# XunshanMan/Object-oriented-SLAM

Hardware: AMD Instinct MI355X
Metric: LM iterations/sec (cams+ellipsoids) (higher is better)
Workload: dtype f64

## Files before the change

object-oriented-slam_amd/csrc/esl_capi.hip:

```cpp
#include <algorithm>
#include <cfloat>
#include <cmath>
#include <cstdio>
#include <cstdlib>
#include <cstring>
#include <numeric>

#include "esl_graph_int.hpp"
#include "esl_graph_layout.hpp"
#include "esl_kernels_map.hpp"
#include "esl_kernels_chunk.hpp"
#include "esl_slam.hpp"
#include "esl_fixed.hpp"

namespace esl {
static thread_local std::string g_err;
void set_error(const std::string& s) { g_err = s; }
}

using namespace esl;

namespace esl {
ProfScope::ProfScope(esl_ctx* ctx, int kind) : c(ctx), slot(-1) {
  if (!c || !c->prof_on) return;
// ... 70 lines not shown
  int n = 0;
  if (hipGetDeviceCount(&n) != hipSuccess) return 0;
  return n;
}

void esl_lm_params_default(esl_lm_params* p) {
  p->max_iters = 10;
  p->max_trials = 10;
  p->tau = 1e-5;
  p->jacobian_mode = ESL_JAC_NUMERIC;
  p->numeric_delta = 1e-9;
  p->linear_solver = ESL_SOLVER_AUTO;
  p->drop_nan_bbox = 1;
  p->bbox_residual = ESL_BBOX_REPROJECTION;
  p->e3d_half_turn = 0;
}

int esl_ctx_create(int device_id, esl_ctx** out) {
  if (!out) return ESL_ERR_INVALID;
  *out = nullptr;
  int n = 0;
  if (hipGetDeviceCount(&n) != hipSuccess || n <= 0) {
    set_error("no HIP device visible: libesl_hip has no CPU fallback");
    return ESL_ERR_NO_DEVICE;
  }
  if (device_id < 0 || device_id >= n) { set_error("device id out of range"); return ESL_ERR_INVALID; }
  ESL_HIP_TRY(hipSetDevice(device_id));
  esl_ctx* c = new esl_ctx();
  c->device = device_id;
  { const char* ov = std::getenv("ESL_CF_OVERLAP"); c->sw_cf_overlap = (ov && ov[0] >= '0' && ov[0] <= '4') ? ov[0] - '0' : 4; }
  { const char* ok = std::getenv("ESL_CF_OS_KERNEL"); c->sw_cf_os_kernel = (ok && ok[0] == '0') ? 0 : 1; }
  { const char* ol = std::getenv("ESL_CF_OS_LIST"); c->sw_cf_os_list = (ol && ol[0] == '0') ? 0 : 1; }
  { const char* sp = std::getenv("ESL_CF_SWEEP"); c->sw_cf_sweep = (sp && sp[0] == '0') ? 0 : 1; }
  { const char* fp = std::getenv("ESL_CF_FWD_PARTS"); const int v = fp ? std::atoi(fp) : 0; if (v == 2 || v == 4 || v == 8) c->sw_cf_fwd_parts = v; }
  { const char* sd = std::getenv("ESL_CF_STRIDE"); const int v = sd ? std::atoi(sd) : 0; c->sw_cf_stride = (v == 16 || v == 32 || v == 48) ? v : 0; }
  auto init = [&]() -> int {
    ESL_HIP_TRY(hipStreamCreateWithFlags(&c->stream, hipStreamNonBlocking));
    ESL_HIP_TRY(hipHostMalloc((void**)&c->host_part, 16 * sizeof(double), hipHostMallocDefault));
    ESL_HIP_TRY(hipMalloc((void**)&c->dev_part, 16 * sizeof(double)));
    ESL_HIP_TRY(hipMalloc((void**)&c->chol_info, 4 * sizeof(int)));
    ESL_HIP_TRY(hipMemset(c->chol_info, 0, 4 * sizeof(int)));
    ESL_HIP_TRY(hipMalloc((void**)&c->tickets, 4 * sizeof(unsigned int)));
    ESL_HIP_TRY(hipMemset(c->tickets, 0, 4 * sizeof(unsigned int)));
    ESL_HIP_TRY(hipMalloc((void**)&c->dev_scal, 8 * sizeof(double)));
    ESL_HIP_TRY(hipEventCreateWithFlags(&c->ev_try, hipEventDisableTiming));
    ESL_HIP_TRY(hipHostMalloc(&c->host_scal, sizeof(LmScalars), hipHostMallocMapped));
    ESL_HIP_TRY(hipHostGetDevicePointer(&c->host_scal_dev, c->host_scal, 0));
    std::memset(c->host_scal, 0, sizeof(LmScalars));
    ESL_HIP_TRY(hipMalloc(&c->lm_dev, 2 * sizeof(LmCore)));
    ESL_HIP_TRY(hipMemset(c->lm_dev, 0, 2 * sizeof(LmCore)));
    ESL_HIP_TRY(hipHostMalloc(&c->lm_host, sizeof(LmHostView), hipHostMallocMapped));
    ESL_HIP_TRY(hipHostGetDevicePointer(&c->lm_host_dev, c->lm_host, 0));
    std::memset(c->lm_host, 0, sizeof(LmHostView));
    return ESL_OK;
  };
  const int rc = init();
  if (rc) { const std::string msg = g_err; esl_ctx_destroy(c); set_error(msg); return rc; }
  *out = c;
  return ESL_OK;
}

int esl_ctx_destroy(esl_ctx* c) {
  if (!c) return ESL_OK;
  (void)hipSetDevice(c->device);
  if (c->stream) (void)hipStreamSynchronize(c->stream);
  slam_sync_side(c);
// ... 763 lines not shown
```

object-oriented-slam_amd/csrc/esl_cf_plan.hpp:

```cpp
#pragma once
#include <algorithm>
#include <array>
#include <cmath>
#include <cstddef>
#include <cstdint>
#include <utility>
#include <vector>

namespace esl {

constexpr int kCfFwdCh = 16;
constexpr int kCfSyT = 128;
constexpr int kCfSegRows = 96;
constexpr int kCfMaxStride = 128;
constexpr int kCfKC = 16;
constexpr int kCfSparseMinCams = 256;

constexpr double kCfUpdFlopsPerMs = 0.83 * 79.0e9;
constexpr double kCfPairMs = (7.82 - 4.21) / (77.35e6 - 31.05e6);
constexpr double kCfSlabMs = 1.30 / 1.35e8;
constexpr double kCfStrideMargin = 0.05;
inline double cf_stride_cost(double upd_flops, double pairs, double slab) {
  return upd_flops / kCfUpdFlopsPerMs + pairs * kCfPairMs + slab * kCfSlabMs;
}
inline int cf_stride_choose(long n_o, const double* upd_flops, const double* pairs, const double* slab) {
  if (n_o < 8192) return kCfFwdCh;
  const double base = cf_stride_cost(upd_flops[0], pairs[0], slab[0]);
  int best = 1;
  double best_ms = base * (1.0 - kCfStrideMargin);
  for (int m = 2; m <= 3; ++m) {
    const double ms = cf_stride_cost(upd_flops[m - 1], pairs[m - 1], slab[m - 1]);
    if (ms < best_ms) { best = m; best_ms = ms; }
  }
  return best * kCfFwdCh;
}

struct CfSwitches {
  int sparse = -1;
  bool tperm_off = false;
  bool no_nd = false;
  int nd_min = 48;
  int stride = 0;
  int os_kernel = 1;
  int os_list = 1;
  int sweep = 1;
};

struct CfSegTables {
  int S = kCfFwdCh, nseg = 0, nw = 0;
  std::vector<int> p, o, first;
  std::vector<int> seg_start, xld, fw_off;
  std::vector<long long> xoff, boff, roff, tw_off;
  int n_fwork = 0, n_twork = 0;
  size_t xc_len = 0, p_blocks = 0, prhs_len = 0;
  double sp_flops = 0;
};
struct CfPlan : CfSegTables {
  int n_list = 0, n_chunks = 0;
  int64_t ldx = 0, ldt = 0, kpad = 0, kpad_s = 0;
  bool nd = false;
  int stride = 0, n_sep = 0, n_seg = 1;
  bool sparse = false;
  int form = 0;
  std::vector<int> os, ou;
  size_t y_len = 0;
  size_t os_npairs = 0;
  bool os_offsets = false;
  double os_flops = 0;
  bool os_list = false;
  std::vector<int> os_run, os_heads;
  size_t osm_npairs = 0, osm_row_npairs = 0, os_list_npairs = 0;
  double osm_flops = 0;
  bool sweep = false;
  std::vector<int> sl_ent;
  size_t xl_len = 0;
  bool tperm = false;
  std::vector<int> rank, unrank, kfirst;
  double upd_flops = 0;
};

inline void cf_entry_lists(int N, int nf, const std::vector<int>& start, const int* cu_start, const int* cu_obj, const int* cu_id,
                           std::vector<int>& os, std::vector<int>& ou) {
  std::vector<int> cur(start.begin(), start.end() - 1);
  os.assign((size_t)start[(size_t)N], 0); ou.assign((size_t)start[(size_t)N], 0);
  for (int sl = 0; sl < nf; ++sl)
    for (int q = cu_start[sl]; q < cu_start[sl + 1]; ++q) { const int at = cur[cu_obj[q]]++; os[(size_t)at] = sl; ou[(size_t)at] = cu_id[q]; }
}
inline CfSegTables cf_walk(int S, int N, int nf, const int* cu_start, const int* cu_obj) {
  CfSegTables t;
  const int nseg = (nf + S - 1) / S;
  t.S = S; t.nseg = nseg; t.nw = (nseg + 63) / 64;
  std::vector<int> last_seg((size_t)N, -1);
  for (int sl = 0; sl < nf; ++sl) {
    const int p = sl / S, pos = sl - p * S;
    if (pos == S - 1) continue;
    for (int q = cu_start[sl]; q < cu_start[sl + 1]; ++q) {
      const int o = cu_obj[q];
      if (last_seg[(size_t)o] != p) { last_seg[(size_t)o] = p; t.p.push_back(p); t.o.push_back(o); t.first.push_back(pos); }
    }
  }
  const size_t n_inc = t.p.size();
  const long long rows = S == kCfFwdCh ? kCfSegRows : 6 * (S - 1);
  t.seg_start.assign((size_t)nseg + 1, 0); t.xld.assign((size_t)nseg, 0); t.fw_off.assign((size_t)nseg + 1, 0);
  t.xoff.assign((size_t)nseg + 1, 0); t.boff.assign((size_t)nseg + 1, 0); t.roff.assign((size_t)nseg + 1, 0); t.tw_off.assign((size_t)nseg + 1, 0);
  for (size_t q = 0; q < n_inc; ++q) ++t.seg_start[(size_t)t.p[q] + 1];
  for (int p = 0; p < nseg; ++p) t.seg_start[(size_t)p + 1] += t.seg_start[(size_t)p];
  for (size_t q = 0; q < n_inc; ++q)
    t.sp_flops += 81.0 * (double)(q - (size_t)t.seg_start[(size_t)t.p[q]] + 1) * (6.0 * (S - 1 - t.first[q]));
// ... 61 lines not shown

inline void cf_os_sides(CfPlan& pl, const std::vector<int>& start) {
  const int S = pl.S;
  const size_t n_inc = pl.p.size();
  pl.os_run.assign(pl.os.size(), 0); pl.os_heads.assign(n_inc, 0);
  std::vector<int> cur(start.begin(), start.end() - 1);
  for (size_t q = 0; q < n_inc; ++q) {
    const int o = pl.o[q], p = pl.p[q], end = start[(size_t)o + 1];
    int k = cur[(size_t)o];
    while (k < end && pl.os[(size_t)k] / S < p) ++k;
    for (int head = -1; k < end && pl.os[(size_t)k] / S == p; ++k) {
      const int sl = pl.os[(size_t)k];
      if (sl % S == S - 1) continue;
      if (head < 0 || pl.os[(size_t)head] != sl) { head = k; ++pl.os_heads[q]; }
      ++pl.os_run[(size_t)head];
    }
    cur[(size_t)o] = k;
  }
  double both = 0, row = 0, brow = 0;
  std::vector<int> v;
  std::vector<std::pair<int, int>> byrank;
  for (int p = 0; p < pl.nseg; ++p) {
    const int q0 = pl.seg_start[(size_t)p], n = pl.seg_start[(size_t)p + 1] - q0;
    v.assign(pl.os_heads.begin() + q0, pl.os_heads.begin() + q0 + n);
    std::sort(v.begin(), v.end());
    for (int i = 0; i < n; ++i) { both += (double)v[(size_t)i] * (double)(n - i); brow += v[(size_t)i]; }
    byrank.clear();
    for (int i = 0; i < n; ++i) { const int o = pl.o[(size_t)(q0 + i)]; byrank.push_back({pl.rank.empty() ? o : pl.rank[(size_t)o], pl.os_heads[(size_t)(q0 + i)]}); }
    std::sort(byrank.begin(), byrank.end());
    for (int i = 0; i < n; ++i) row += (double)byrank[(size_t)i].second * (double)(i + 1);
  }
  pl.osm_npairs = (size_t)(both + brow); pl.osm_row_npairs = (size_t)(row + brow);
  pl.osm_flops = 2.0 * 6.0 * (81.0 * both + 9.0 * brow);
}

inline bool cf_plan_build(int N, int nf, size_t EU, const std::vector<int>& start, const int* cu_start, const int* cu_obj, const int* cu_id, bool chain_ok,
                          bool comm, size_t total_mem, const CfSwitches& sw, CfPlan& pl) {
  pl = CfPlan{};
  const size_t nfz = (size_t)nf, n_o = (size_t)9 * N;
  const int nch = (nf + kCfFwdCh - 1) / kCfFwdCh;
  pl.ldx = (int64_t)((n_o + 1 + 127) / 128 * 128);
  pl.kpad = (int64_t)((6 * nfz + kCfKC - 1) / kCfKC * kCfKC);
  pl.ldt = pl.ldx;
  pl.n_list = start[(size_t)N]; pl.n_chunks = nch;
  pl.nseg = nch; pl.nw = (nch + 63) / 64;
  if ((size_t)std::max(N, 1) * (size_t)(nch + 1) > ((size_t)1 << 28)) return false;
  cf_entry_lists(N, nf, start, cu_start, cu_obj, cu_id, pl.os, pl.ou);
  CfSegTables& seg = pl;
  if (chain_ok && nf >= kCfSparseMinCams && N > 0 && (size_t)nch * (size_t)(N + 1) <= ((size_t)1 << 28) && !sw.no_nd) {
    seg = cf_walk(kCfFwdCh, N, nf, cu_start, cu_obj);
    const double dense = (double)n_o * (double)n_o * 6.0 * (double)nfz;
    const double sparse = (double)n_o * (double)n_o * 6.0 * (double)(nfz / kCfFwdCh) + 24.0 * pl.sp_flops;
    pl.sparse = sw.sparse >= 0 ? sw.sparse != '0' : (n_o >= 2048 && sparse < 0.5 * dense);
    const double need = 8.0 * (81.0 * (double)pl.p_blocks + (double)pl.xc_len + 2.0 * (double)pl.ldt * (double)n_o +
                               2.0 * 6.0 * (double)(nfz / kCfFwdCh) * (double)pl.ldx  + 54.0 * (double)EU );
    pl.form = sw.sparse == '2' || need > 0.4 * (double)total_mem ? 2 : 1;
    if ((sw.sparse < 0 || sw.sparse == '3') && !comm) pl.form = 3;
  }
  const bool sp = pl.sparse;
  std::vector<int> first_cam;
  pl.tperm = sp && N > 0 && !sw.tperm_off;
  if (pl.tperm) {
    std::vector<int> cnt(nfz + 2, 0);
    first_cam.assign((size_t)N, nf);
    for (int o = 0; o < N; ++o) if (start[(size_t)o + 1] > start[(size_t)o]) first_cam[(size_t)o] = pl.os[(size_t)start[(size_t)o]];
    for (int o = 0; o < N; ++o) ++cnt[(size_t)first_cam[(size_t)o] + 1];
// ... 18 lines not shown
      seg = std::move(cand[want / kCfFwdCh - 1]);
    }
    if (!want) want = kCfFwdCh;
    if (want != pl.S) seg = cf_walk(want, N, nf, cu_start, cu_obj);
  }
  pl.nd = nfz >= (size_t)std::max(sw.nd_min, 2 * kCfFwdCh) && !sw.no_nd;
  if (pl.nd) {
    int sd = 16 * (int)std::max(1.0, std::floor(std::sqrt((double)nfz) / 16.0 + 0.5));
    sd = std::min(sd, kCfMaxStride);
    if (sp) sd = pl.S;
    pl.stride = sd; pl.n_sep = nf / sd; pl.n_seg = (nf + sd - 1) / sd;
  }
  if (sp) pl.kpad_s = (int64_t)((6 * (size_t)pl.n_sep + kCfKC - 1) / kCfKC * kCfKC);
  if (pl.tperm) pl.upd_flops = cf_staircase(pl.S, N, nf, pl.unrank, first_cam, pl.kfirst);
  if (sp && pl.form == 3) {
    const CfOsCounts n = cf_os_counts(pl.S, N, start, pl.os, pl.rank);
    const size_t y_recs = std::max<size_t>(pl.p.size(), 1) * (size_t)(pl.S - 1);
    pl.os_flops = 2.0 * 6.0 * (81.0 * n.prod + 9.0 * n.rhs_entries);
    pl.os_npairs = (size_t)(n.prod + n.rhs_entries);
    pl.y_len = y_recs * 54 + std::max<size_t>(nfz, 1) * 6;
    pl.os_offsets = sw.os_kernel != 0 && 54 * std::max(EU, y_recs) <= (size_t)INT32_MAX;
    cf_os_sides(pl, start);
    pl.os_list = sw.os_list != 0;
    pl.os_list_npairs = pl.os_list ? pl.osm_npairs : pl.os_npairs;
    pl.sweep = sw.sweep != 0;
    if (pl.sweep) {
      std::vector<int> cur(start.begin(), start.end() - 1);
      pl.sl_ent.assign((size_t)cu_start[nf], 0);
      for (int sl = 0; sl < nf; ++sl)
        for (int q = cu_start[sl]; q < cu_start[sl + 1]; ++q) pl.sl_ent[(size_t)q] = cur[cu_obj[q]]++;
      long long cols = 0;
      for (int x : pl.xld) cols += x;
      pl.xl_len = 6 * (size_t)cols;
    }
  }
  return true;
}

}
```

object-oriented-slam_amd/csrc/esl_cf_sweep.hpp:

```cpp
#pragma once
#include "esl_cf.hpp"

namespace esl {

constexpr int kCfSweepSI = 3 * kCfFwdCh - 1;

#define CF_LT(r, c) ((r) * ((r) + 1) / 2 + (c))
__device__ __forceinline__ void cf_chol6(double (&d)[21], double (&is)[6], bool& ok) {
#pragma unroll
  for (int j = 0; j < 6; ++j) {
    const double p = d[CF_LT(j, j)];
    ok = ok && (p > 0);
    double q = __builtin_amdgcn_rsq(p);
    q = q * (1.5 - 0.5 * p * q * q);
    q = q * (1.5 - 0.5 * p * q * q);
    is[j] = q;
    d[CF_LT(j, j)] = p * q;
#pragma unroll
    for (int r = j + 1; r < 6; ++r) d[CF_LT(r, j)] *= q;
#pragma unroll
    for (int r = j + 1; r < 6; ++r)
#pragma unroll
      for (int c = j + 1; c <= r; ++c) d[CF_LT(r, c)] -= d[CF_LT(r, j)] * d[CF_LT(c, j)];
  }
}

static __global__ __launch_bounds__(64) void k_cf_twist(int nf_all, int stride, const double* __restrict__ Hcc, double lambda,
                                                        const double* __restrict__ Lfac, const double* __restrict__ Gfac,
                                                        double* __restrict__ Pm, double* __restrict__ Qm, int* __restrict__ info) {
  __shared__ double sH[kCfSweepSI * 36], sG[kCfSweepSI * 36], sL[kCfSweepSI * 21];
  const int lane = threadIdx.x;
  const int beg = (int)blockIdx.x * stride;
  const int len = ((beg + stride - 1 < nf_all) ? beg + stride - 1 : nf_all) - beg;
  if (len <= 0) return;
  {
    constexpr int kQ = (kCfSweepSI * 36 + 63) / 64, kL = (kCfSweepSI * 21 + 63) / 64;
    double th[kQ], tg[kQ], tl[kL];
#pragma unroll
// ... 365 lines not shown
          for (int q = 0; q < 6; ++q) t += P[a * 6 + q] * d[q];
          sv[(ii * 6 + a) * 64 + lane] = t;
        }
      }
      if (on) {
        const bool rmw = __any(s_first < s_last && s_first < p0 + hl && p0 < s_last) != 0;
#pragma unroll
        for (int q0 = 0; q0 < CH * 6; q0 += 8) {
          double t[8], old[8];
#pragma unroll
          for (int e = 0; e < 8; ++e) t[e] = sv[((q0 + e < hl * 6) ? q0 + e : 0) * 64 + lane];
          if (rmw) {
#pragma unroll
            for (int e = 0; e < 8; ++e) {
              const int q = q0 + e, pos = p0 + q / 6;
              old[e] = (q < hl * 6 && pos >= s_first && pos < s_last) ? dst[(size_t)pos * dstep + q % 6] : 0.0;
            }
          } else {
#pragma unroll
            for (int e = 0; e < 8; ++e) old[e] = 0.0;
          }
#pragma unroll
          for (int e = 0; e < 8; ++e) {
            const int q = q0 + e, pos = p0 + q / 6;
            if (q < hl * 6 && pos < s_last) dst[(size_t)pos * dstep + q % 6] = (pos >= s_first) ? old[e] + t[e] : t[e];
          }
        }
      }
      __builtin_amdgcn_wave_barrier();
    }
  }
}

static __global__ __launch_bounds__(64) void k_cf_wxo(int stride, const int* __restrict__ sl_start, const int* __restrict__ sl_ent,
                                                      const int* __restrict__ sl_obj, const double* __restrict__ V, const double* __restrict__ vy,
                                                      const double* __restrict__ xo, double* __restrict__ z) {
  __shared__ double red[64];
  const int i = blockIdx.x, lane = threadIdx.x;
  if (i % stride == stride - 1) return;
  const int l = lane < 54 ? lane : 0, b = l / 6;
  const int qa = sl_start[i], qb = sl_start[i + 1];
  double s = 0;
  for (int q = qa; q < qb; q += 4) {
    double v[4], w[4];
#pragma unroll
    for (int e = 0; e < 4; ++e) {
      const int qq = (q + e < qb) ? q + e : qa;
      v[e] = V[(size_t)sl_ent[qq] * 54 + l];
      w[e] = xo[(size_t)9 * sl_obj[qq] + b];
    }
#pragma unroll
    for (int e = 0; e < 4; ++e) if (q + e < qb) s += v[e] * w[e];
  }
  red[lane] = s;
  __builtin_amdgcn_wave_barrier();
  if (lane < 6) {
    double t = 0;
#pragma unroll
    for (int bb = 0; bb < 9; ++bb) t += red[6 * bb + lane];
    z[(size_t)i * 6 + lane] = vy[(size_t)i * 6 + lane] - t;
  }
}
static __global__ __launch_bounds__(64) void k_cf_z_fwd(int nf_all, int stride, const double* __restrict__ Mm, double* __restrict__ z) {
  __shared__ double sM[kCfSweepSI * 36], sz[kCfSweepSI * 6];
  const int lane = threadIdx.x;
  const int beg = (int)blockIdx.x * stride;
// ... 33 lines not shown
```

object-oriented-slam_amd/csrc/esl_ctx.hpp:

```cpp
#pragma once
#include <hip/hip_runtime.h>

#include <cstdint>
#include <string>
#include <type_traits>
#include <vector>

#include "../../include/esl.h"
#include "esl_cf_plan.hpp"
#include "esl_math.hpp"

namespace esl {

void set_error(const std::string& s);
#define ESL_HIP_TRY(expr)                                                                         \
  do {                                                                                            \
    hipError_t _e = (expr);                                                                       \
    if (_e != hipSuccess) {                                                                       \
      esl::set_error(std::string(#expr) + ": " + hipGetErrorString(_e));                          \
      return ESL_ERR_HIP;                                                                         \
    }                                                                                             \
  } while (0)

struct DevGraph {
// ... 192 lines not shown
  void* lm_dev = nullptr;
  void* lm_host = nullptr;
  void* lm_host_dev = nullptr;
  void* host_scal = nullptr;
  void* host_scal_dev = nullptr;
  bool sys_combined = false;
  void* comm = nullptr;
  int comm_ranks = 1, comm_rank = 0;
  bool comm_replicated = false;
  esl_host_allreduce_fn host_allreduce = nullptr;
  void* host_user = nullptr;
  double* host_stage = nullptr;
  double* dev_gather = nullptr;
  double* host_gather = nullptr;
  double* Linv_ws = nullptr;
  double* z_ws = nullptr;
  int64_t S_lda = 0;
  bool cf_chain_ok = false;
  bool cf_ready = false;
  bool cf_unavailable = false;
  esl::CfPlan cf_plan;
  int *cf_oe_start = nullptr, *cf_oe_u = nullptr, *cf_oe_slot = nullptr, *cf_od_start = nullptr, *cf_od_edge = nullptr, *cf_oe_cst = nullptr;
  double *cf_Linv = nullptr, *cf_M = nullptr, *cf_N = nullptr, *cf_V = nullptr, *cf_vy = nullptr, *cf_z = nullptr;
  double *cf_B = nullptr, *cf_Lfac = nullptr, *cf_G = nullptr;
  double *cf_Zt = nullptr, *cf_Hs = nullptr, *cf_Bs = nullptr, *cf_LfacS = nullptr, *cf_GS = nullptr, *cf_LiS = nullptr, *cf_MS = nullptr,
         *cf_NS = nullptr, *cf_R = nullptr;
  double *cf_Xt = nullptr, *cf_T = nullptr, *cf_Linv_ws = nullptr, *cf_part = nullptr;
  int *cf_seg_start = nullptr, *cf_seg_obj = nullptr, *cf_seg_first = nullptr, *cf_cmap = nullptr, *cf_xld = nullptr, *cf_fwork = nullptr, *cf_twork = nullptr;
  unsigned long long* cf_mask = nullptr;
  long long *cf_xoff = nullptr, *cf_boff = nullptr, *cf_roff = nullptr;
  double *cf_Xc = nullptr, *cf_Xs = nullptr, *cf_P = nullptr, *cf_Prhs = nullptr, *cf_Y = nullptr, *cf_Yr = nullptr;
  double *cf_Pm = nullptr, *cf_Qm = nullptr, *cf_XL = nullptr;
  int* cf_sl_ent = nullptr;
  long long* cf_os_start = nullptr;
  int *cf_os_cnt = nullptr, *cf_os_pairs = nullptr;
  int *cf_os_run = nullptr, *cf_os_heads = nullptr;
  double* cf_Vm = nullptr;
  int *cf_rank = nullptr, *cf_unrank = nullptr, *cf_kfirst = nullptr;
  double* cf_xo_t = nullptr;
  int lm_solver_used = 0;
  bool fx_on = false;
  std::vector<uint8_t> fx_flags;
  esl::AnchGraph fx;
  char* fx_blob = nullptr; size_t fx_blob_cap = 0;
  double* fx_A = nullptr; double* fx_chi = nullptr;
  std::vector<int> fx_bb_map, fx_e3_map;
  std::vector<int> fx_grav_obj;
  bool chain_ok = false;
  esl::Scratch chain_ws;
  esl_pcg_params pcg = {1000, 8, 1e-10};
  esl_pcg_params pcg_run = {1000, 8, 1e-10};
  double* pcg_ws = nullptr; size_t pcg_ws_cap = 0;
  double* pcg_st = nullptr; double* pcg_M = nullptr;
  double* pcg_host = nullptr;
  bool pcg_ran = false;
  bool pcg_reset = true;
  void* chol_rt = nullptr;
  void* chol_prof_scope = nullptr;
  unsigned long long graph_fp = 0;
  bool repl_checked = false;
  double *chol_pack = nullptr, *chol_pack2 = nullptr;
  size_t chol_pack_len = 0;
  bool schur_attr_set = false;
  int sw_chol_dist = -1;
  bool sw_chol_overlap = true;
  int sw_cf_overlap = 4;
  int sw_cf_os_kernel = 1;
  int sw_cf_os_list = 1;
  int sw_cf_fwd_parts = 8;
  int sw_cf_sweep = 1;
  int sw_cf_stride = 0;
};
```

object-oriented-slam_amd/csrc/esl_slam.hip:

```cpp
#include "esl_slam.hpp"

#include <algorithm>
#include <array>
#include <chrono>
#include <cmath>
#include <cstdio>
#include <cstdlib>
#include <cstring>

#include "esl_cf.hpp"
#include "esl_cf_sweep.hpp"
#include "esl_chol.hpp"
#include "esl_fixed.hpp"
#include "esl_kernels_slam.hpp"
#include "esl_pcg.hpp"

namespace esl {

static __global__ __launch_bounds__(256) void k_cf_updates(DevGraph g, int nb_obj, double lambda, const double* __restrict__ objs, const double* __restrict__ bo,
                                                           const double* __restrict__ xo, double* __restrict__ objs_trial, double* __restrict__ obj_part,
                                                           const double* __restrict__ cams, const double* __restrict__ xc, const double* __restrict__ bc,
                                                           double* __restrict__ cams_trial, double* __restrict__ cam_part) {
  if ((int)blockIdx.x < nb_obj) cf_obj_update_one(g, lambda, objs, bo, xo, objs_trial, obj_part, blockIdx.x * 256 + threadIdx.x);
  else slam_cam_update_one(g, lambda, cams, xc, bc, cams_trial, cam_part, ((int)blockIdx.x - nb_obj) * 256 + threadIdx.x);
// ... 208 lines not shown
  if (c->sw_chol_overlap) {
    d.pack2 = c->chol_pack2;
    d.bcast_on = [](void* u, double* dev, size_t count, int root, hipStream_t st) { return comm_bcast((esl_ctx*)u, dev, count, root, st); };
  }
  return ESL_OK;
}
static bool cf_applicable(const esl_ctx* c) { return c->cf_chain_ok && (!c->comm || c->comm_replicated); }
static bool cf_dist(const esl_ctx* c) {
  if (!c->comm || !c->comm_replicated || c->comm_ranks < 2) return false;
  if (c->sw_chol_dist >= 0) return c->sw_chol_dist == 1;
  return 9L * c->g.n_objs >= 8192;
}
static bool chain_applicable(const esl_ctx* c) { return c->chain_ok && c->g.n_ue == 0 && !c->comm; }
static int slam_pick_solver(const esl_ctx* c) {
  const int want = c->lm.p.linear_solver;
  if (want == ESL_SOLVER_PCG) return c->comm ? -3 : ESL_SOLVER_PCG;
  if (want == ESL_SOLVER_CAMERA_CHAIN) return chain_applicable(c) ? ESL_SOLVER_CAMERA_CHAIN : -2;
  if (want == ESL_SOLVER_AUTO && c->fx_on && chain_applicable(c)) return ESL_SOLVER_CAMERA_CHAIN;
  if (want == ESL_SOLVER_REDUCED_CAMERA) return ESL_SOLVER_REDUCED_CAMERA;
  if (want == ESL_SOLVER_REDUCED_ELLIPSOID) return cf_applicable(c) ? ESL_SOLVER_REDUCED_ELLIPSOID : -1;
  if (!cf_applicable(c) || c->cf_unavailable) return ESL_SOLVER_REDUCED_CAMERA;
  const double nc = (double)c->S_n, no = 9.0 * c->g.n_objs;
  return (no * no * nc + no * no * no / 3.0 < nc * nc * nc / 3.0) ? ESL_SOLVER_REDUCED_ELLIPSOID : ESL_SOLVER_REDUCED_CAMERA;
}
static void cf_forget(esl_ctx* c) {
  c->cf_oe_start = c->cf_oe_u = c->cf_oe_slot = c->cf_oe_cst = nullptr;
  c->cf_seg_start = c->cf_seg_obj = c->cf_seg_first = c->cf_cmap = c->cf_xld = c->cf_fwork = c->cf_twork = nullptr;
  c->cf_mask = nullptr; c->cf_xoff = c->cf_boff = c->cf_roff = nullptr;
  c->cf_Linv = c->cf_M = c->cf_N = c->cf_V = c->cf_B = c->cf_Lfac = c->cf_G = c->cf_vy = c->cf_z = nullptr;
  c->cf_T = c->cf_Linv_ws = c->cf_part = nullptr;
  c->cf_Zt = c->cf_Hs = c->cf_Bs = c->cf_LfacS = c->cf_GS = c->cf_LiS = c->cf_MS = c->cf_NS = c->cf_R = nullptr;
  c->cf_Xc = c->cf_Xs = c->cf_P = c->cf_Prhs = c->cf_Xt = c->cf_Y = c->cf_Yr = nullptr;
  c->cf_os_start = nullptr; c->cf_os_cnt = c->cf_os_pairs = c->cf_os_run = c->cf_os_heads = nullptr; c->cf_Vm = nullptr;
  c->cf_Pm = c->cf_Qm = c->cf_XL = nullptr; c->cf_sl_ent = nullptr;
  c->cf_rank = c->cf_unrank = c->cf_kfirst = nullptr; c->cf_xo_t = nullptr;
  c->cf_plan = CfPlan{};
  c->cf_ready = false;
}
static int cf_ensure_impl(esl_ctx* c);
static int cf_ensure(esl_ctx* c) {
  if (c->cf_ready) return ESL_OK;
  const int rc = cf_ensure_impl(c);
  if (rc) { cf_forget(c); (void)hipGetLastError(); return rc; }
  c->cf_ready = true;
  return ESL_OK;
}
static_assert(kCfKC == kKC, "esl_cf_plan.hpp pads K to the rank-K update's chunk");
static int cf_ensure_impl(esl_ctx* c) {
  const DevGraph& g = c->g;
  const int N = g.n_objs, nfi = g.n_free_cams;
  const size_t nf = (size_t)nfi, EU = (size_t)g.n_bbox + g.n_e3d, n_o = (size_t)9 * N;
  const bool timing = std::getenv("ESL_UPLOAD_HOST_TIMING") != nullptr;
  const double t0 = timing ? now_us() : 0;
  CfSwitches sw;
  { const char* e = std::getenv("ESL_CF_SPARSE"); sw.sparse = e ? (int)(unsigned char)e[0] : -1; }
  { const char* e = std::getenv("ESL_CF_TPERM"); sw.tperm_off = e && e[0] == '0'; }
  sw.no_nd = std::getenv("ESL_CF_NO_ND") != nullptr;
  static const int nd_min = [] { const char* e = std::getenv("ESL_CF_ND_MIN"); return e ? std::atoi(e) : 48; }();
  sw.nd_min = nd_min; sw.stride = c->sw_cf_stride; sw.os_kernel = c->sw_cf_os_kernel; sw.os_list = c->sw_cf_os_list;
  sw.sweep = c->sw_cf_sweep;
  size_t free_b = 0, total_b = 0;
  if (nfi >= kCfSparseMinCams) ESL_HIP_TRY(hipMemGetInfo(&free_b, &total_b));
  CfPlan& pl = c->cf_plan;
  if (!cf_plan_build(N, nfi, EU, c->h_ue_start, c->h_cu_start, c->h_cu_obj, c->h_cu_id, c->cf_chain_ok, c->comm != nullptr, total_b, sw, pl)) {
    set_error("camera-first elimination: the (ellipsoid, camera chunk) range table of this graph exceeds 1 GB");
    return ESL_ERR_ALLOC;
  }
  const bool sp = pl.sparse, os3 = sp && pl.form == 3, osm = os3 && pl.os_list;
  const bool swp = os3 && pl.sweep;
  const int nch = pl.n_chunks, nseg = pl.nseg, nw = pl.nw, N1 = N + 1;
  const size_t n_inc = pl.p.size();
  const size_t y_recs = std::max<size_t>(n_inc, 1) * (size_t)(pl.S - 1), nb = (size_t)N * (N + 1) / 2 + N;
  const double t1 = timing ? now_us() : 0;
  BlobStage st;
  struct Up { int item; const void* src; size_t bytes; };
  std::vector<Up> ups;
  auto ship = [&](auto** dst, const auto& v) { ups.push_back({st.up(dst, v.size()), v.data(), v.size() * sizeof(v[0])}); };
  ship(&c->cf_oe_start, c->h_ue_start); ship(&c->cf_oe_u, pl.ou); ship(&c->cf_oe_slot, pl.os);
  int* d_inc = nullptr; int* d_fw_off = nullptr; long long* d_tw_off = nullptr;
  int i_inc = -1;
  if (pl.tperm) { ship(&c->cf_rank, pl.rank); ship(&c->cf_unrank, pl.unrank); ship(&c->cf_kfirst, pl.kfirst); }
  if (sp) {
    i_inc = st.up(&d_inc, 4 * n_inc); ship(&c->cf_seg_start, pl.seg_start); ship(&c->cf_xld, pl.xld);
    ship(&c->cf_xoff, pl.xoff); ship(&c->cf_boff, pl.boff); ship(&c->cf_roff, pl.roff); ship(&d_fw_off, pl.fw_off); ship(&d_tw_off, pl.tw_off);
  }
  if (osm) { ship(&c->cf_os_run, pl.os_run); ship(&c->cf_os_heads, pl.os_heads); }
  if (swp) ship(&c->cf_sl_ent, pl.sl_ent);
  st.work(&c->cf_oe_cst, (size_t)std::max(N, 1) * (nch + 1));
  if (sp) {
    st.work(&c->cf_cmap, (size_t)nseg * N1); st.work(&c->cf_mask, (size_t)N1 * nw); st.work(&c->cf_seg_obj, n_inc); st.work(&c->cf_seg_first, n_inc);
    st.work(&c->cf_fwork, 2 * (size_t)pl.n_fwork); st.work(&c->cf_twork, 3 * (size_t)pl.n_twork);
  }
  st.work(&c->cf_Linv, nf * 36); st.work(&c->cf_M, nf * 36); st.work(&c->cf_N, nf * 36); st.work(&c->cf_V, EU * 54);
  st.work(&c->cf_B, nf * 36); st.work(&c->cf_Lfac, nf * 21); st.work(&c->cf_G, nf * 36); st.work(&c->cf_vy, nf * 6); st.work(&c->cf_z, nf * 6);
  st.work(&c->cf_T, (size_t)pl.ldt * n_o); st.work(&c->cf_Linv_ws, ((n_o + kNB - 1) / kNB) * kNB * kNB);
  if (pl.tperm) st.work(&c->cf_xo_t, n_o);
  if (n_o <= 1024) st.work(&c->cf_part, (size_t)kCholMaxSplit * (size_t)pl.ldt * n_o);
  if (pl.nd) {
    const size_t ns = (size_t)std::max(pl.n_sep, 1);
    st.work(&c->cf_Zt, nf * 36); st.work(&c->cf_Hs, ns * 36); st.work(&c->cf_Bs, ns * 36); st.work(&c->cf_LfacS, ns * 21);
    st.work(&c->cf_GS, ns * 36); st.work(&c->cf_LiS, ns * 36); st.work(&c->cf_MS, ns * 36); st.work(&c->cf_NS, ns * 36);
    st.work(&c->cf_R, ns * 6 * (size_t)pl.ldx);
  }
  if (sp) {
    if (!swp) st.work(&c->cf_Xc, pl.xc_len);
    st.work(&c->cf_Xs, (size_t)pl.ldx * (size_t)pl.kpad_s);
    if (pl.form == 1) { st.work(&c->cf_P, pl.p_blocks * 81); st.work(&c->cf_Prhs, pl.prhs_len); }
    if (pl.form == 3) {
      st.work(&c->cf_Y, y_recs * 54); st.work(&c->cf_Yr, std::max<size_t>(nf, 1) * 6);
      st.work(&c->cf_os_start, nb + 1); st.work(&c->cf_os_cnt, nb); st.work(&c->cf_os_pairs, 2 * std::max<size_t>(pl.os_list_npairs, 1));
      if (osm) st.work(&c->cf_Vm, EU * 54);
      if (swp) { st.work(&c->cf_Pm, nf * 36); st.work(&c->cf_Qm, nf * 36); st.work(&c->cf_XL, std::max<size_t>(pl.xl_len, 1)); }
    }
  } else {
    st.work(&c->cf_Xt, (size_t)pl.ldx * (size_t)pl.kpad);
  }
  if (int rc = st.reserve(c->arena_solve)) return rc;
  for (const Up& u : ups) if (u.bytes) std::memcpy(st.host<char>(u.item), u.src, u.bytes);
  if (sp && n_inc) {
    int* inc = st.host<int>(i_inc);
// ... 106 lines not shown
                       c->cf_Linv, st);
  }
  int slabs(bool beside) {
    auto twist = [&](hipStream_t s) {
      hipLaunchKernelGGL(k_cf_twist, dim3((unsigned)nseg), dim3(64), 0, s, nf, st, c->Hcc, lambda, c->cf_Lfac, c->cf_G, c->cf_Pm, c->cf_Qm, c->chol_info);
    };
    hipError_t e_tw = hipSuccess;
    segment_chains([&] {
      if (!swp) return;
      if (!beside) { twist(main); return; }
      e_tw = hipEventRecord(rt.cf_ev_c, main);
      if (e_tw == hipSuccess) e_tw = hipStreamWaitEvent(rt.cf_side, rt.cf_ev_c, 0);
      if (e_tw != hipSuccess) return;
      join.armed = true;
      twist(rt.cf_side);
      e_tw = hipEventRecord(rt.cf_ev_t, rt.cf_side);
    });
    ESL_HIP_TRY(e_tw);
    if (beside) {
      ESL_HIP_TRY(hipEventRecord(rt.cf_ev_a, main));
      ESL_HIP_TRY(hipStreamWaitEvent(rt.cf_side, rt.cf_ev_a, 0));
      join.armed = true;
    }
    sep_chain(beside ? rt.cf_side : main);
    if (beside) ESL_HIP_TRY(hipEventRecord(rt.cf_ev_s, rt.cf_side));
    if (swp) {
      edge_scale(beside ? 1 : 0, main);
      if (beside) ESL_HIP_TRY(hipStreamWaitEvent(main, rt.cf_ev_t, 0));
      auto sweep = [&](auto parts) {
        hipLaunchKernelGGL((k_cf_sweep<decltype(parts)::value>), dim3((unsigned)pl.n_fwork), dim3(64), 0, main, nf, n_o, pl.n_chunks, c->cf_oe_cst, c->cf_oe_slot,
                           c->cf_V, c->cf_vy, c->cf_M, (const double*)c->cf_Zt, c->cf_Pm, c->cf_Qm, c->cf_R, ldx, st, segs(), c->cf_Y, c->cf_Yr, c->cf_XL,
                           (long long)(st == kCfFwdCh ? kCfSegRows : 6 * (st - 1)));
      };
      if (c->sw_cf_fwd_parts == 8) sweep(std::integral_constant<int, 8>{});
      else if (c->sw_cf_fwd_parts == 4) sweep(std::integral_constant<int, 4>{});
      else sweep(std::integral_constant<int, 2>{});
      return ESL_OK;
    }
    edge_scale(beside ? 1 : 0, main);
    auto forward = [&](auto parts) {
      hipLaunchKernelGGL((k_cf_forward<2, decltype(parts)::value>), dim3((unsigned)pl.n_fwork), dim3(64), 0, main, nf, n_o, pl.n_chunks, c->cf_oe_cst, c->cf_oe_slot,
                         c->cf_V, c->cf_vy, c->cf_M, c->cf_Xc, ldx, st, st - 1, (const double*)c->cf_Zt, c->cf_R, st, segs());
    };
    if (c->sw_cf_fwd_parts == 8) forward(std::integral_constant<int, 8>{});
    else if (c->sw_cf_fwd_parts == 4) forward(std::integral_constant<int, 4>{});
    else forward(std::integral_constant<int, 2>{});
    return ESL_OK;
  }
  void sep_rhs(hipStream_t s, bool sp = true) const {
    hipLaunchKernelGGL(k_cf_sep_rhs, dim3(cg, (unsigned)ns), dim3(64), 0, s, nf, n_o, st, pl.n_chunks, c->cf_oe_cst, c->cf_oe_slot, c->cf_V, c->cf_vy,
                       c->cf_G, c->cf_LiS, sp ? c->cf_Xc : c->cf_Xt, ldx, c->cf_R, sp ? (const int*)c->cf_cmap : nullptr, sp ? segs() : CfSegs{},
                       (const double*)(sp && swp ? c->cf_XL : nullptr), (long long)(st == kCfFwdCh ? kCfSegRows : 6 * (st - 1)));
  }
  void sep_forward(hipStream_t s, bool sp = true) const {
    hipLaunchKernelGGL(k_cf_forward<1>, dim3(cg), dim3(64), 0, s, ns, n_o, pl.n_chunks, c->cf_oe_cst, c->cf_oe_slot, c->cf_V, c->cf_vy,
                       c->cf_MS, sp ? c->cf_Xs : c->cf_Xt, ldx, ns, ns, (const double*)nullptr, c->cf_R, sp ? 0 : st, CfSegs{});
  }
  void products(hipStream_t s) const {
    hipLaunchKernelGGL(k_cf_seg_syrk, dim3((unsigned)pl.n_twork), dim3(256), 0, s, c->cf_twork, c->cf_seg_start, c->cf_seg_first, c->cf_xoff,
                       c->cf_xld, c->cf_Xc, c->cf_boff, c->cf_P);
    hipLaunchKernelGGL(k_cf_seg_rhs, dim3((unsigned)pl.n_fwork), dim3(64), 0, s, c->cf_fwork, c->cf_seg_start, c->cf_xoff, c->cf_xld, c->cf_Xc,
                       c->cf_roff, c->cf_Prhs);
  }
  void gather_products(long c_begin, long c_end, int accumulate) const {
    int o2b, o2e;
    const dim3 grid = block_grid(c_begin, c_end, o2b, o2e);
    hipLaunchKernelGGL(k_cf_T_gather, grid, dim3(256), 0, main, N, pl.nw, c->cf_mask, c->cf_cmap, c->cf_boff, c->cf_roff, c->cf_P, c->cf_Prhs,
// ... 794 lines not shown
```

Before: 19.62.

## Add paired-column sweep kernel so each lane solves two right-hand-side columns

Adds k_cf_sweep_pair, in which each lane handles two columns of the segment's right-hand side (128 columns per 64-lane block), plus a host-built work list mapping blocks to (segment, column group). The aim is to reuse each shared-memory load of the M/Z/P/Q 6x6 blocks across two columns, halving block count and matrix staging traffic per column. The cost is doubled register state per lane (x, acc, u, erec arrays), which may reduce occupancy or cause spills, plus extra shared memory for the interleaved sv buffer. It is enabled by default (sweep_cols=2) whenever the sweep path is active.

```diff
diff --git a/object-oriented-slam_amd/csrc/esl_capi.hip b/object-oriented-slam_amd/csrc/esl_capi.hip
--- a/object-oriented-slam_amd/csrc/esl_capi.hip
+++ b/object-oriented-slam_amd/csrc/esl_capi.hip
@@ -126,6 +126,7 @@
   { const char* ok = std::getenv("ESL_CF_OS_KERNEL"); c->sw_cf_os_kernel = (ok && ok[0] == '0') ? 0 : 1; }
   { const char* ol = std::getenv("ESL_CF_OS_LIST"); c->sw_cf_os_list = (ol && ol[0] == '0') ? 0 : 1; }
   { const char* sp = std::getenv("ESL_CF_SWEEP"); c->sw_cf_sweep = (sp && sp[0] == '0') ? 0 : 1; }
+  { const char* sc = std::getenv("ESL_CF_SWEEP_COLS"); c->sw_cf_sweep_cols = (sc && sc[0] == '1') ? 1 : 2; }
   { const char* fp = std::getenv("ESL_CF_FWD_PARTS"); const int v = fp ? std::atoi(fp) : 0; if (v == 2 || v == 4 || v == 8) c->sw_cf_fwd_parts = v; }
   { const char* sd = std::getenv("ESL_CF_STRIDE"); const int v = sd ? std::atoi(sd) : 0; c->sw_cf_stride = (v == 16 || v == 32 || v == 48) ? v : 0; }
   auto init = [&]() -> int {
diff --git a/object-oriented-slam_amd/csrc/esl_cf_plan.hpp b/object-oriented-slam_amd/csrc/esl_cf_plan.hpp
--- a/object-oriented-slam_amd/csrc/esl_cf_plan.hpp
+++ b/object-oriented-slam_amd/csrc/esl_cf_plan.hpp
@@ -10,6 +10,7 @@
 namespace esl {
 
 constexpr int kCfFwdCh = 16;
+constexpr int kCfPairCols = 128;
 constexpr int kCfSyT = 128;
 constexpr int kCfSegRows = 96;
 constexpr int kCfMaxStride = 128;
@@ -44,6 +45,7 @@
   int os_kernel = 1;
   int os_list = 1;
   int sweep = 1;
+  int sweep_cols = 2;
 };
 
 struct CfSegTables {
@@ -74,6 +76,8 @@
   bool sweep = false;
   std::vector<int> sl_ent;
   size_t xl_len = 0;
+  std::vector<int> pw_off, pwork;
+  int n_pwork = 0;
   bool tperm = false;
   std::vector<int> rank, unrank, kfirst;
   double upd_flops = 0;
@@ -201,6 +205,17 @@
   }
   pl.osm_npairs = (size_t)(both + brow); pl.osm_row_npairs = (size_t)(row + brow);
   pl.osm_flops = 2.0 * 6.0 * (81.0 * both + 9.0 * brow);
+}
+
+inline void cf_pair_work(const std::vector<int>& seg_start, std::vector<int>& pw_off, std::vector<int>& pwork) {
+  const size_t nseg = seg_start.empty() ? 0 : seg_start.size() - 1;
+  pw_off.assign(nseg + 1, 0); pwork.clear();
+  for (size_t p = 0; p < nseg; ++p) {
+    const int m = 9 * (seg_start[p + 1] - seg_start[p]) + 1;
+    const int ng = (m + kCfPairCols - 1) / kCfPairCols;
+    pw_off[p + 1] = pw_off[p] + ng;
+    for (int q = 0; q < ng; ++q) { pwork.push_back((int)p); pwork.push_back(q); }
+  }
 }
 
 inline bool cf_plan_build(int N, int nf, size_t EU, const std::vector<int>& start, const int* cu_start, const int* cu_obj, const int* cu_id, bool chain_ok,
@@ -285,6 +300,8 @@
       long long cols = 0;
       for (int x : pl.xld) cols += x;
       pl.xl_len = 6 * (size_t)cols;
+      if (sw.sweep_cols == 2) cf_pair_work(pl.seg_start, pl.pw_off, pl.pwork);
+      pl.n_pwork = (int)(pl.pwork.size() / 2);
     }
   }
   return true;
diff --git a/object-oriented-slam_amd/csrc/esl_cf_sweep.hpp b/object-oriented-slam_amd/csrc/esl_cf_sweep.hpp
--- a/object-oriented-slam_amd/csrc/esl_cf_sweep.hpp
+++ b/object-oriented-slam_amd/csrc/esl_cf_sweep.hpp
@@ -4,6 +4,7 @@
 namespace esl {
 
 constexpr int kCfSweepSI = 3 * kCfFwdCh - 1;
+constexpr int kCfPairE = 4;
 
 #define CF_LT(r, c) ((r) * ((r) + 1) / 2 + (c))
 __device__ __forceinline__ void cf_chol6(double (&d)[21], double (&is)[6], bool& ok) {
@@ -435,6 +436,283 @@
   }
 }
 
+template <int PARTS>
+static __global__ __launch_bounds__(64) void k_cf_sweep_pair(int nf_all, int n_o, int n_chunks, const int* __restrict__ oe_cst, const int* __restrict__ oe_slot,
+                                                             const double* __restrict__ V, const double* __restrict__ vy, const double* __restrict__ Mm,
+                                                             const double* __restrict__ Zt, const double* __restrict__ Pm, const double* __restrict__ Qm,
+                                                             double* __restrict__ R, long ldx, int stride, CfSegs sg, const int* __restrict__ pwork,
+                                                             double* __restrict__ Y, double* __restrict__ Yr, double* __restrict__ XL, long long xl_rows) {
+  static_assert(PARTS == 2 || PARTS == 4 || PARTS == 8, "halves, quarters or eighths of a chunk");
+  constexpr int CH = kCfFwdCh / PARTS;
+  constexpr int HC = kCfFwdCh / 2;
+  constexpr int kQ = (HC * 36 + 63) / 64;
+  constexpr int kB = 2;
+  constexpr int kE = kCfPairE;
+  static_assert(HC % CH == 0 && HC * 6 <= 64, "a part lies inside a half chunk; one load per lane stages its right-hand sides");
+  __shared__ __attribute__((aligned(16))) double sA[HC * 36], sB[HC * 36], sP[HC * 36];
+  __shared__ double sv[CH * 6 * 128];
+  __shared__ double svy[HC * 6];
+  const int lane = threadIdx.x;
+  const int seg = pwork[2 * blockIdx.x];
+  auto jc = [&](int c) { return pwork[2 * blockIdx.x + 1] * kCfPairCols + 64 * c + lane; };
+  const int ob = sg.seg_start[seg];
+  const int jr = 9 * (sg.seg_start[seg + 1] - ob);
+  const int SI = stride - 1;
+  const int beg = seg * stride;
+  const int nf = (beg + SI < nf_all) ? beg + SI : nf_all;
+  if (beg >= nf) return;
+  const int len = nf - beg;
+  const bool use_z = Zt != nullptr && seg >= 1;
+  int oc[2], ka[2], s_first[2], s_last[2], t_first[2], ecnt[2], eslot[2][kE];
+  int kind[2];
+  double* dst[2];
+  double erec[2][kE][6];
+#pragma unroll
+  for (int c = 0; c < 2; ++c) {
+    const int j = jc(c);
+    kind[c] = j < jr ? 1 : j == jr ? 2 : 0;
+    const int oi = j < jr ? j / 9 : 0, b = j - 9 * oi;
+    const int o = j < jr ? sg.seg_obj[ob + oi] : 0;
+    const int* cst = oe_cst + (size_t)o * (n_chunks + 1);
+    oc[c] = o;
+    s_first[c] = len; s_last[c] = -1; t_first[c] = len; ecnt[c] = 0; ka[c] = 0;
+#pragma unroll
+    for (int e = 0; e < kE; ++e) {
+      eslot[c][e] = -1;
+#pragma unroll
+      for (int a = 0; a < 6; ++a) erec[c][e][a] = 0.0;
+    }
+    if (kind[c] == 2) { s_first[c] = 0; s_last[c] = len - 1; }
+    else if (kind[c] == 1) {
+      const int c0 = beg / kCfFwdCh, c1 = (c0 + stride / kCfFwdCh < n_chunks) ? c0 + stride / kCfFwdCh : n_chunks;
+      const int k0 = cst[c0], kb = cst[c1];
+      if (k0 < kb) {
+        const int f = oe_slot[k0] - beg;
+        int k = kb - 1, l = oe_slot[k] - beg;
+        while (l >= len && k > k0) { --k; l = oe_slot[k] - beg; }
+        if (f < len) {
+          s_first[c] = f; s_last[c] = l; ecnt[c] = k - k0 + 1; ka[c] = k0;
+          if (ecnt[c] > kE) t_first[c] = oe_slot[k0 + kE] - beg;
+#pragma unroll
+          for (int e = 0; e < kE; ++e) {
+            const int kk = e < ecnt[c] ? k0 + e : k0;
+            eslot[c][e] = oe_slot[kk] - beg;
+            const double* src = V + ((size_t)kk * 9 + b) * 6;
+#pragma unroll
+            for (int a = 0; a < 6; ++a) erec[c][e][a] = src[a];
+          }
+        }
+      }
+    }
+    dst[c] = kind[c] == 2 ? Yr + (size_t)beg * 6 : Y + ((size_t)(ob + oi) * SI) * 54 + b * 6;
+  }
+  auto gather = [&](int h0, int p0, int hl) {
+#pragma unroll
+    for (int q = 0; q < CH * 6 * 2; ++q) sv[q * 64 + lane] = 0.0;
+    __builtin_amdgcn_wave_barrier();
+#pragma unroll
+    for (int c = 0; c < 2; ++c) {
+      if (kind[c] == 2) {
+#pragma unroll
+        for (int q = 0; q < CH * 6; ++q) sv[(2 * q + c) * 64 + lane] = (q < hl * 6) ? svy[h0 * 6 + q] : 0.0;
+      } else if (kind[c] == 1) {
+#pragma unroll
+        for (int e = 0; e < kE; ++e) {
+          const int at = eslot[c][e] - p0;
+          if (e < ecnt[c] && at >= 0 && at < hl) {
+#pragma unroll
+            for (int a = 0; a < 6; ++a) sv[(2 * (at * 6 + a) + c) * 64 + lane] += erec[c][e][a];
+          }
+        }
+        if (t_first[c] < p0 + hl && s_last[c] >= p0) {
+          const int kb = ka[c] + ecnt[c], b = jc(c) % 9;
+          for (int k = ka[c] + kE; k < kb; k += kB) {
+            int sl[kB];
+            double rec[kB][6];
+#pragma unroll
+            for (int e = 0; e < kB; ++e) {
+              const int kk = (k + e < kb) ? k + e : ka[c];
+              sl[e] = oe_slot[kk];
+              const double* src = V + ((size_t)kk * 9 + b) * 6;
+#pragma unroll
+              for (int a = 0; a < 6; ++a) rec[e][a] = src[a];
+            }
+#pragma unroll
+            for (int e = 0; e < kB; ++e) {
+              const int at = sl[e] - beg - p0;
+              if (k + e < kb && at >= 0 && at < hl) {
+#pragma unroll
+                for (int a = 0; a < 6; ++a) sv[(2 * (at * 6 + a) + c) * 64 + lane] += rec[e][a];
+              }
+            }
+          }
+        }
+      }
+    }
+    __builtin_amdgcn_wave_barrier();
+  };
+  double x[2][6] = {{0, 0, 0, 0, 0, 0}, {0, 0, 0, 0, 0, 0}}, acc[2][6] = {{0, 0, 0, 0, 0, 0}, {0, 0, 0, 0, 0, 0}};
+  for (int i0 = beg; i0 < nf; i0 += HC) {
+    const int clen = (nf - i0 < HC) ? nf - i0 : HC;
+    if (!__any((kind[0] && s_first[0] < i0 - beg + clen) || (kind[1] && s_first[1] < i0 - beg + clen))) continue;
+    __builtin_amdgcn_wave_barrier();
+    {
+      double tm[kQ], tz[kQ], tp[kQ];
+#pragma unroll
+      for (int q = 0; q < kQ; ++q) {
+        const int idx = q * 64 + lane, cl = idx < clen * 36 ? idx : 0;
+        tm[q] = Mm[(size_t)i0 * 36 + cl];
+        tz[q] = use_z ? Zt[(size_t)i0 * 36 + cl] : 0.0;
+        tp[q] = Pm[(size_t)i0 * 36 + cl];
+      }
+      const double ty = vy[(size_t)i0 * 6 + (lane < clen * 6 ? lane : 0)];
+#pragma unroll
+      for (int q = 0; q < kQ; ++q) if (q * 64 + lane < HC * 36) { sA[q * 64 + lane] = tm[q]; sB[q * 64 + lane] = tz[q]; sP[q * 64 + lane] = tp[q]; }
+      if (lane < HC * 6) svy[lane] = ty;
+    }
+    __builtin_amdgcn_wave_barrier();
+    for (int h0 = 0; h0 < clen; h0 += CH) {
+      const int hl = (clen - h0 < CH) ? clen - h0 : CH;
+      const int p0 = i0 - beg + h0;
+      if (!__any((kind[0] && s_first[0] < p0 + hl) || (kind[1] && s_first[1] < p0 + hl))) continue;
+      gather(h0, p0, hl);
+      for (int ii = 0; ii < hl; ++ii) {
+        const double* M = sA + (h0 + ii) * 36;
+        double xn[2][6];
+#pragma unroll
+        for (int a = 0; a < 6; ++a) {
+          double t0 = sv[(2 * (ii * 6 + a) + 0) * 64 + lane], t1 = sv[(2 * (ii * 6 + a) + 1) * 64 + lane];
+#pragma unroll
+          for (int q = 0; q < 6; ++q) { const double m = M[a * 6 + q]; t0 -= m * x[0][q]; t1 -= m * x[1][q]; }
+          xn[0][a] = t0; xn[1][a] = t1;
+        }
+#pragma unroll
+        for (int a = 0; a < 6; ++a) { x[0][a] = xn[0][a]; x[1][a] = xn[1][a]; }
+        if (use_z) {
+          const double* Z = sB + (h0 + ii) * 36;
+#pragma unroll
+          for (int a = 0; a < 6; ++a)
+#pragma unroll
+            for (int q = 0; q < 6; ++q) { const double m = Z[q * 6 + a]; acc[0][a] += m * xn[0][q]; acc[1][a] += m * xn[1][q]; }
+        }
+        const double* P = sP + (h0 + ii) * 36;
+#pragma unroll
+        for (int a = 0; a < 6; ++a) {
+          double t0 = 0, t1 = 0;
+#pragma unroll
+          for (int q = 0; q < 6; ++q) { const double m = P[a * 6 + q]; t0 += m * xn[0][q]; t1 += m * xn[1][q]; }
+          sv[(2 * (ii * 6 + a) + 0) * 64 + lane] = t0; sv[(2 * (ii * 6 + a) + 1) * 64 + lane] = t1;
+        }
+      }
+#pragma unroll
+      for (int c = 0; c < 2; ++c) {
+        if (kind[c] == 0) continue;
+#pragma unroll
+        for (int ii = 0; ii < CH; ++ii) {
+          double t[6];
+#pragma unroll
+          for (int a = 0; a < 6; ++a) t[a] = sv[(2 * ((ii < hl ? ii : 0) * 6 + a) + c) * 64 + lane];
+          const int pos = p0 + ii;
+          if (ii < hl && pos >= s_first[c]) {
+            double2* d = reinterpret_cast<double2*>(dst[c] + (size_t)pos * (kind[c] == 2 ? 6 : 54));
+#pragma unroll
+            for (int a = 0; a < 3; ++a) d[a] = make_double2(t[2 * a], t[2 * a + 1]);
+          }
+        }
+      }
+      __builtin_amdgcn_wave_barrier();
+    }
+  }
+#pragma unroll
+  for (int c = 0; c < 2; ++c) {
+    if (use_z && kind[c]) {
+      const long tcol = kind[c] == 2 ? (long)n_o : 9L * (sg.rank ? sg.rank[oc[c]] : oc[c]) + jc(c) % 9;
+#pragma unroll
+      for (int a = 0; a < 6; ++a) R[(size_t)tcol + (size_t)(6 * (seg - 1) + a) * (size_t)ldx] = acc[c][a];
+    }
+    if (kind[c] && len == SI) {
+      double* xl = XL + (size_t)(sg.xoff[seg] / xl_rows) * 6 + (size_t)jc(c);
+      const size_t ld = (size_t)sg.xld[seg];
+#pragma unroll
+      for (int a = 0; a < 6; ++a) xl[(size_t)a * ld] = x[c][a];
+    }
+  }
+  double u[2][6] = {{0, 0, 0, 0, 0, 0}, {0, 0, 0, 0, 0, 0}};
+  for (int i0 = beg + ((len - 1) / HC) * HC; i0 >= beg; i0 -= HC) {
+    const int clen = (nf - i0 < HC) ? nf - i0 : HC;
+    if (!__any((kind[0] && s_last[0] >= i0 - beg) || (kind[1] && s_last[1] >= i0 - beg))) continue;
+    __builtin_amdgcn_wave_barrier();
+    {
+      double tq[kQ], tp[kQ];
+#pragma unroll
+      for (int q = 0; q < kQ; ++q) {
+        const int idx = q * 64 + lane, cl = idx < clen * 36 ? idx : 0;
+        tq[q] = Qm[(size_t)i0 * 36 + cl];
+        tp[q] = Pm[(size_t)i0 * 36 + cl];
+      }
+      const double ty = vy[(size_t)i0 * 6 + (lane < clen * 6 ? lane : 0)];
+#pragma unroll
+      for (int q = 0; q < kQ; ++q) if (q * 64 + lane < HC * 36) { sA[q * 64 + lane] = tq[q]; sP[q * 64 + lane] = tp[q]; }
+      if (lane < HC * 6) svy[lane] = ty;
+    }
+    __builtin_amdgcn_wave_barrier();
+    for (int h0 = ((clen - 1) / CH) * CH; h0 >= 0; h0 -= CH) {
+      const int hl = (clen - h0 < CH) ? clen - h0 : CH;
+      const int p0 = i0 - beg + h0;
+      if (!__any((kind[0] && s_last[0] >= p0) || (kind[1] && s_last[1] >= p0))) continue;
+      gather(h0, p0, hl);
+      for (int ii = hl - 1; ii >= 0; --ii) {
+        const double* Qi = sA + (h0 + ii) * 36;
+        const bool both0 = p0 + ii >= s_first[0], both1 = p0 + ii >= s_first[1];
+        double un[2][6], d[2][6];
+#pragma unroll
+        for (int a = 0; a < 6; ++a) {
+          const double v0 = sv[(2 * (ii * 6 + a) + 0) * 64 + lane], v1 = sv[(2 * (ii * 6 + a) + 1) * 64 + lane];
+          double t0 = v0, t1 = v1;
+#pragma unroll
+          for (int q = 0; q < 6; ++q) { const double m = Qi[a * 6 + q]; t0 -= m * u[0][q]; t1 -= m * u[1][q]; }
+          un[0][a] = t0; un[1][a] = t1;
+          d[0][a] = both0 ? t0 - v0 : t0; d[1][a] = both1 ? t1 - v1 : t1;
+        }
+#pragma unroll
+        for (int a = 0; a < 6; ++a) { u[0][a] = un[0][a]; u[1][a] = un[1][a]; }
+        const double* P = sP + (h0 + ii) * 36;
+#pragma unroll
+        for (int a = 0; a < 6; ++a) {
+          double t0 = 0, t1 = 0;
+#pragma unroll
+          for (int q = 0; q < 6; ++q) { const double m = P[a * 6 + q]; t0 += m * d[0][q]; t1 += m * d[1][q]; }
+          sv[(2 * (ii * 6 + a) + 0) * 64 + lane] = t0; sv[(2 * (ii * 6 + a) + 1) * 64 + lane] = t1;
+        }
+      }
+      const bool rmw = __any((s_first[0] < s_last[0] && s_first[0] < p0 + hl && p0 < s_last[0]) ||
+                             (s_first[1] < s_last[1] && s_first[1] < p0 + hl && p0 < s_last[1])) != 0;
+#pragma unroll
+      for (int c = 0; c < 2; ++c) {
+        if (kind[c] == 0) continue;
+#pragma unroll
+        for (int ii = 0; ii < CH; ++ii) {
+          double t[6];
+          double2 old[3];
+#pragma unroll
+          for (int a = 0; a < 6; ++a) t[a] = sv[(2 * ((ii < hl ? ii : 0) * 6 + a) + c) * 64 + lane];
+          const int pos = p0 + ii;
+          double2* d = reinterpret_cast<double2*>(dst[c] + (size_t)pos * (kind[c] == 2 ? 6 : 54));
+          const bool add = pos >= s_first[c];
+          if (ii < hl && pos < s_last[c]) {
+#pragma unroll
+            for (int a = 0; a < 3; ++a) old[a] = (rmw && add) ? d[a] : make_double2(0.0, 0.0);
+#pragma unroll
+            for (int a = 0; a < 3; ++a)
+              d[a] = add ? make_double2(old[a].x + t[2 * a], old[a].y + t[2 * a + 1]) : make_double2(t[2 * a], t[2 * a + 1]);
+          }
+        }
+      }
+      __builtin_amdgcn_wave_barrier();
+    }
+  }
+}
+
 static __global__ __launch_bounds__(64) void k_cf_wxo(int stride, const int* __restrict__ sl_start, const int* __restrict__ sl_ent,
                                                       const int* __restrict__ sl_obj, const double* __restrict__ V, const double* __restrict__ vy,
                                                       const double* __restrict__ xo, double* __restrict__ z) {
diff --git a/object-oriented-slam_amd/csrc/esl_ctx.hpp b/object-oriented-slam_amd/csrc/esl_ctx.hpp
--- a/object-oriented-slam_amd/csrc/esl_ctx.hpp
+++ b/object-oriented-slam_amd/csrc/esl_ctx.hpp
@@ -248,6 +248,7 @@
   double *cf_Xc = nullptr, *cf_Xs = nullptr, *cf_P = nullptr, *cf_Prhs = nullptr, *cf_Y = nullptr, *cf_Yr = nullptr;
   double *cf_Pm = nullptr, *cf_Qm = nullptr, *cf_XL = nullptr;
   int* cf_sl_ent = nullptr;
+  int* cf_pwork = nullptr;
   long long* cf_os_start = nullptr;
   int *cf_os_cnt = nullptr, *cf_os_pairs = nullptr;
   int *cf_os_run = nullptr, *cf_os_heads = nullptr;
@@ -285,5 +286,6 @@
   int sw_cf_os_list = 1;
   int sw_cf_fwd_parts = 8;
   int sw_cf_sweep = 1;
+  int sw_cf_sweep_cols = 2;
   int sw_cf_stride = 0;
 };
diff --git a/object-oriented-slam_amd/csrc/esl_slam.hip b/object-oriented-slam_amd/csrc/esl_slam.hip
--- a/object-oriented-slam_amd/csrc/esl_slam.hip
+++ b/object-oriented-slam_amd/csrc/esl_slam.hip
@@ -264,7 +264,7 @@
   c->cf_Zt = c->cf_Hs = c->cf_Bs = c->cf_LfacS = c->cf_GS = c->cf_LiS = c->cf_MS = c->cf_NS = c->cf_R = nullptr;
   c->cf_Xc = c->cf_Xs = c->cf_P = c->cf_Prhs = c->cf_Xt = c->cf_Y = c->cf_Yr = nullptr;
   c->cf_os_start = nullptr; c->cf_os_cnt = c->cf_os_pairs = c->cf_os_run = c->cf_os_heads = nullptr; c->cf_Vm = nullptr;
-  c->cf_Pm = c->cf_Qm = c->cf_XL = nullptr; c->cf_sl_ent = nullptr;
+  c->cf_Pm = c->cf_Qm = c->cf_XL = nullptr; c->cf_sl_ent = c->cf_pwork = nullptr;
   c->cf_rank = c->cf_unrank = c->cf_kfirst = nullptr; c->cf_xo_t = nullptr;
   c->cf_plan = CfPlan{};
   c->cf_ready = false;
@@ -290,7 +290,7 @@
   sw.no_nd = std::getenv("ESL_CF_NO_ND") != nullptr;
   static const int nd_min = [] { const char* e = std::getenv("ESL_CF_ND_MIN"); return e ? std::atoi(e) : 48; }();
   sw.nd_min = nd_min; sw.stride = c->sw_cf_stride; sw.os_kernel = c->sw_cf_os_kernel; sw.os_list = c->sw_cf_os_list;
-  sw.sweep = c->sw_cf_sweep;
+  sw.sweep = c->sw_cf_sweep; sw.sweep_cols = c->sw_cf_sweep_cols;
   size_t free_b = 0, total_b = 0;
   if (nfi >= kCfSparseMinCams) ESL_HIP_TRY(hipMemGetInfo(&free_b, &total_b));
   CfPlan& pl = c->cf_plan;
@@ -318,6 +318,7 @@
   }
   if (osm) { ship(&c->cf_os_run, pl.os_run); ship(&c->cf_os_heads, pl.os_heads); }
   if (swp) ship(&c->cf_sl_ent, pl.sl_ent);
+  if (swp && pl.n_pwork) ship(&c->cf_pwork, pl.pwork);
   st.work(&c->cf_oe_cst, (size_t)std::max(N, 1) * (nch + 1));
   if (sp) {
     st.work(&c->cf_cmap, (size_t)nseg * N1); st.work(&c->cf_mask, (size_t)N1 * nw); st.work(&c->cf_seg_obj, n_inc); st.work(&c->cf_seg_first, n_inc);
@@ -490,7 +491,16 @@
                            c->cf_V, c->cf_vy, c->cf_M, (const double*)c->cf_Zt, c->cf_Pm, c->cf_Qm, c->cf_R, ldx, st, segs(), c->cf_Y, c->cf_Yr, c->cf_XL,
                            (long long)(st == kCfFwdCh ? kCfSegRows : 6 * (st - 1)));
       };
-      if (c->sw_cf_fwd_parts == 8) sweep(std::integral_constant<int, 8>{});
+      auto sweep_pair = [&](auto parts) {
+        hipLaunchKernelGGL((k_cf_sweep_pair<decltype(parts)::value>), dim3((unsigned)pl.n_pwork), dim3(64), 0, main, nf, n_o, pl.n_chunks, c->cf_oe_cst,
+                           c->cf_oe_slot, c->cf_V, c->cf_vy, c->cf_M, (const double*)c->cf_Zt, c->cf_Pm, c->cf_Qm, c->cf_R, ldx, st, segs(),
+                           (const int*)c->cf_pwork, c->cf_Y, c->cf_Yr, c->cf_XL, (long long)(st == kCfFwdCh ? kCfSegRows : 6 * (st - 1)));
+      };
+      if (pl.n_pwork) {
+        if (c->sw_cf_fwd_parts == 8) sweep_pair(std::integral_constant<int, 8>{});
+        else if (c->sw_cf_fwd_parts == 4) sweep_pair(std::integral_constant<int, 4>{});
+        else sweep_pair(std::integral_constant<int, 2>{});
+      } else if (c->sw_cf_fwd_parts == 8) sweep(std::integral_constant<int, 8>{});
       else if (c->sw_cf_fwd_parts == 4) sweep(std::integral_constant<int, 4>{});
       else sweep(std::integral_constant<int, 2>{});
       return ESL_OK;
```

New measurement: 19.75 (median of 6 runs). About the same (+0.7%).
